# zju3dv/pats

Hardware: AMD Instinct MI355X
Metric: image-pairs/sec (coarse+fine OT) on 640x480 MegaDepth; OT iters/sec per pair (higher is better)
Workload: dtype f32 (contractions: fp32 operands split into fp16 hi + lo, three exact-product MFMA passes, fp32 accumulate)

## Files before the change

### pats_amd/csrc/gather.hip

```cpp
#include "common.hpp"

#include <cstdlib>
#include <type_traits>

namespace pats {

template <int POL, typename T>
__device__ __forceinline__ T ldm(const T* p) {
    if (POL & 1) return __builtin_nontemporal_load(p);
    return *p;
}
template <int POL, typename T>
__device__ __forceinline__ void stm(T* p, T v) {
    if (POL & 2) __builtin_nontemporal_store(v, p);
    else *p = v;
}

typedef float f2u __attribute__((ext_vector_type(2), aligned(4)));
template <int POL>
__device__ __forceinline__ f2u ldm2(const float* p) {
    const f2u* q = reinterpret_cast<const f2u*>(p);
    if (POL & 1) return __builtin_nontemporal_load(q);
    return *q;
}

template <int DT> struct map_elem { using type = uint16_t; };
template <> struct map_elem<PATS_MAP_F32> { using type = float; };
template <int DT> using map_t = typename map_elem<DT>::type;

template <int DT>
__device__ __forceinline__ float widen(uint32_t h) {
    if (DT == PATS_MAP_BF16) return __uint_as_float(h << 16);
    return (float)__builtin_bit_cast(_Float16, (uint16_t)h);
}
template <int DT>
__device__ __forceinline__ float widen_hi(uint32_t h) {
    if (DT == PATS_MAP_BF16) return __uint_as_float(h & 0xffff0000u);
    return (float)__builtin_bit_cast(_Float16, (uint16_t)(h >> 16));
}
typedef uint32_t u32u __attribute__((aligned(2)));
template <int POL>
__device__ __forceinline__ uint32_t ldh2(const uint16_t* p) {
    const u32u* q = reinterpret_cast<const u32u*>(p);
    if (POL & 1) return __builtin_nontemporal_load(q);
    return *q;
}
typedef uint32_t u4 __attribute__((ext_vector_type(4)));
typedef float f2s __attribute__((ext_vector_type(2), aligned(4)));
template <int POL>
__device__ __forceinline__ void stm2(float* p, f2s v) {
    f2s* q = reinterpret_cast<f2s*>(p);
    if (POL & 2) __builtin_nontemporal_store(v, q);
    else *q = v;
}

template <int OT> using out_t = map_t<OT>;
template <int OT>
__device__ __forceinline__ out_t<OT> narrow(float v) {
    if constexpr (OT == PATS_MAP_F32) return v;
    else if constexpr (OT == PATS_MAP_F16) return __builtin_bit_cast(uint16_t, (_Float16)v);
    else return __builtin_bit_cast(uint16_t, (__bf16)v);
}
template <int OT>
__device__ __forceinline__ uint32_t narrow2(float lo, float hi) {
    return (uint32_t)narrow<OT>(lo) | ((uint32_t)narrow<OT>(hi) << 16);
}
template <int POL>
__device__ __forceinline__ void sth2(uint16_t* p, uint32_t v) {
    u32u* q = reinterpret_cast<u32u*>(p);
    if (POL & 2) __builtin_nontemporal_store(v, q);
    else *q = v;
}
template <int OT>
__device__ __forceinline__ u4 narrow8(const float* t) {
    typedef float f4 __attribute__((ext_vector_type(4)));
    const f4 a = *reinterpret_cast<const f4*>(t), b = *reinterpret_cast<const f4*>(t + 4);
    u4 r;
    r.x = narrow2<OT>(a.x, a.y); r.y = narrow2<OT>(a.z, a.w);
    r.z = narrow2<OT>(b.x, b.y); r.w = narrow2<OT>(b.z, b.w);
    return r;
}

template <int DT, int POL>
__device__ __forceinline__ float pooled_tap(const map_t<DT>* q, int row) {
    if constexpr (DT == PATS_MAP_F32) {
        const f2u a = ldm2<POL>(q), c2 = ldm2<POL>(q + row);
        return (((a.x + a.y) + c2.x) + c2.y) / 4.0f;
    } else {
        const uint32_t a = ldh2<POL>(q), c2 = ldh2<POL>(q + row);
        return (((widen<DT>(a) + widen_hi<DT>(a)) + widen<DT>(c2)) + widen_hi<DT>(c2)) / 4.0f;
    }
}
template <int DT, int POL>
__device__ __forceinline__ float single_tap(const map_t<DT>* q) {
    if constexpr (DT == PATS_MAP_F32) return ldm<POL>(q);
    else return widen<DT>(ldm<POL>(q));
}

template <int DT, int POL, int OT>
__global__ void __launch_bounds__(256)
fine_desc_kernel(const map_t<DT>* __restrict__ f0, const map_t<DT>* __restrict__ f1,
                 const map_t<DT>* __restrict__ f2, const float* __restrict__ title,
                 const float* __restrict__ rubbish, int64_t B, out_t<OT>* __restrict__ desc,
                 const int64_t* __restrict__ B_live) {
    const int64_t n = blockIdx.x;
    const int64_t b = n % B;
    if (B_live && b >= *B_live) return;
    const int lane = threadIdx.x & 63, wave = threadIdx.x >> 6;
    out_t<OT>* o = desc + n * 264 * 145;
    int pt[3], off0[3], off1[3];
    bool live[3];
#pragma unroll
    for (int g = 0; g < 3; ++g) {
        const int p = OT == PATS_MAP_F32 ? lane + 64 * g : (g < 2 ? 2 * lane + g : 128 + lane);
        live[g] = p < 145;
        pt[g] = p < 144 ? p : 0;
        const int r = pt[g] / 12, c = pt[g] - r * 12;
        off0[g] = (4 * r + 1) * 48 + 4 * c + 1;
        off1[g] = (2 * r) * 24 + 2 * c;
    }
    const bool dust = lane == 16;
    auto put = [&](int ch, float v0, float v1, float v2) {
        out_t<OT>* row = o + ch * 145;
        if constexpr (OT == PATS_MAP_F32) {
            stm<POL>(row + lane, v0);
            stm<POL>(row + lane + 64, v1);
            if (live[2]) stm<POL>(row + lane + 128, dust ? rubbish[b * 264 + ch] : v2);
        } else {
            sth2<POL>(row + 2 * lane, narrow2<OT>(v0, v1));
            if (live[2]) stm<POL>(row + lane + 128, narrow<OT>(dust ? rubbish[b * 264 + ch] : v2));
        }
    };
    for (int ch = wave; ch < 8; ch += 4) {
        const float v = title[b * 8 + ch];
        put(ch, v, v, v);
    }
#pragma unroll 2
    for (int ch = 8 + wave; ch < 72; ch += 4) {
        const map_t<DT>* m = f0 + (n * 64 + (ch - 8)) * 48 * 48;
        float v[3];
#pragma unroll
        for (int g = 0; g < 3; ++g) v[g] = pooled_tap<DT, POL>(m + off0[g], 48);
        put(ch, v[0], v[1], v[2]);
    }
#pragma unroll 2
    for (int ch = 72 + wave; ch < 136; ch += 4) {
        const map_t<DT>* m = f1 + (n * 64 + (ch - 72)) * 24 * 24;
        float v[3];
#pragma unroll
        for (int g = 0; g < 3; ++g) v[g] = pooled_tap<DT, POL>(m + off1[g], 24);
        put(ch, v[0], v[1], v[2]);
    }
#pragma unroll 4
    for (int ch = 136 + wave; ch < 264; ch += 4) {
        const map_t<DT>* m = f2 + (n * 128 + (ch - 136)) * 144;
        put(ch, single_tap<DT, POL>(m + pt[0]), single_tap<DT, POL>(m + pt[1]), single_tap<DT, POL>(m + pt[2]));
    }
}

__device__ __forceinline__ long long round_half_even_div(float x, float d) {
    return (long long)rintf(x / d);
}

struct third_point {
    long long i00[2], bb2, i2;
};
__device__ __forceinline__ third_point third_point_at(const float* __restrict__ mk0, const float* __restrict__ mk1,
                                                      int64_t p, int64_t b, int64_t B, bool write,
                                                      int64_t* __restrict__ ps_out, int64_t* __restrict__ pt_out) {
    constexpr int W = 8, M = 52;
    const long long s0 = round_half_even_div(mk0[p * 2 + 0], 4.0f) * 4, s1 = round_half_even_div(mk0[p * 2 + 1], 4.0f) * 4;
    float t0 = mk1[p * 2 + 0], t1 = mk1[p * 2 + 1];
    t0 = t0 >= 96.f ? 96.f : t0; t1 = t1 >= 96.f ? 96.f : t1;
    t0 = t0 <= 0.f ? 0.f : t0;   t1 = t1 <= 0.f ? 0.f : t1;
    const long long q0 = round_half_even_div(t0, 4.0f) * 4, q1 = round_half_even_div(t1, 4.0f) * 4;
    if (write) {
        if (ps_out) { ps_out[p * 2] = s0; ps_out[p * 2 + 1] = s1; }
        if (pt_out) { pt_out[p * 2] = q0; pt_out[p * 2 + 1] = q1; }
    }
    auto fdiv2 = [](long long v) { return v >= 0 ? v / 2 : -((-v + 1) / 2); };
    third_point r;
    r.i00[0] = b * M * M + (fdiv2(s1) - W / 2 + 2) * M + (fdiv2(s0) - W / 2 + 2);
    r.i00[1] = b * M * M + (fdiv2(q1) - W / 2 + 2) * M + (fdiv2(q0) - W / 2 + 2);
    long long i2 = b * 144 + round_half_even_div((float)s1, 8.0f) * 12 + round_half_even_div((float)s0, 8.0f);
    i2 = i2 < 0 ? 0 : (i2 > B * 144 - 1 ? B * 144 - 1 : i2);
    r.bb2 = i2 / 144;
    r.i2 = i2 - r.bb2 * 144;
    return r;
}

template <int POL, int OT>
__global__ void __launch_bounds__(256)
third_desc_point_kernel(const float* __restrict__ ff0, const float* __restrict__ ff1,
                  const float* __restrict__ mk0, const float* __restrict__ mk1,
                  const int64_t* __restrict__ b_ids, const float* __restrict__ kenc,
                  const float* __restrict__ rubbish, int64_t P, int64_t B,
                  out_t<OT>* __restrict__ out0, out_t<OT>* __restrict__ out1, int64_t* __restrict__ ps_out,
                  int64_t* __restrict__ pt_out, const int64_t* __restrict__ P_dev) {
    constexpr int W = 8, M = 52, C = 128;
    int64_t live = P;
    if (P_dev) { const int64_t n = *P_dev; live = n < P ? n : P; }
    const int64_t per = (live + 7) >> 3, p = (int64_t)(blockIdx.x & 7) * per + (blockIdx.x >> 3);
    if ((int64_t)(blockIdx.x >> 3) >= per || p >= live) return;
    const int lane = threadIdx.x & 63, wave = threadIdx.x >> 6;
    const int64_t b = b_ids[p];
    const third_point tp = third_point_at(mk0, mk1, p, b, B, threadIdx.x == 0, ps_out, pt_out);
    const int wx = lane % W, wy = lane / W;
    long long i0 = tp.i00[0] + wy * M + wx, i1 = tp.i00[1] + wy * M + wx;
    const long long lim = B * M * M - 1;
    i0 = i0 < 0 ? 0 : (i0 > lim ? lim : i0);
    i1 = i1 < 0 ? 0 : (i1 > lim ? lim : i1);
    const long long bb0 = i0 / (M * M), r0 = i0 - bb0 * (M * M);
    const long long bb1 = i1 / (M * M), r1 = i1 - bb1 * (M * M);
    out_t<OT>* o0 = out0 + p * C * 65;
    out_t<OT>* o1 = out1 + p * C * 65;
    const float* src0 = ff0 + bb0 * C * (M * M) + r0;
    const float* src1 = ff1 + bb1 * C * (M * M) + r1;
#pragma unroll 1
    for (int c0 = 32 * wave; c0 < 32 * wave + 32; c0 += 8) {
        float a[8], c[8], ke[8];
#pragma unroll
        for (int k = 0; k < 8; ++k) {
            a[k] = ldm<POL>(src0 + (int64_t)(c0 + k) * (M * M));
            c[k] = ldm<POL>(src1 + (int64_t)(c0 + k) * (M * M));
            ke[k] = kenc[(c0 + k) * 64 + lane];
        }
#pragma unroll
        for (int k = 0; k < 8; ++k) {
            stm<POL>(o0 + (c0 + k) * 65 + lane, narrow<OT>(a[k] + ke[k]));
            stm<POL>(o1 + (c0 + k) * 65 + lane, narrow<OT>(c[k] + ke[k]));
        }
    }
    if (lane < 32) {
        const int ch = 32 * wave + lane;
        const float rb = rubbish[(tp.bb2 * C + ch) * 144 + tp.i2];
        o0[ch * 65 + 64] = narrow<OT>(rb);
        o1[ch * 65 + 64] = narrow<OT>(rb);
    }
}

constexpr int THIRD_TILE = 8;

template <int POL>
__global__ void __launch_bounds__(256)
third_desc_kernel(const float* __restrict__ ff0, const float* __restrict__ ff1,
                  const float* __restrict__ mk0, const float* __restrict__ mk1,
                  const int64_t* __restrict__ b_ids, const float* __restrict__ kenc,
                  const float* __restrict__ rubbish, int64_t P, int64_t B,
                  float* __restrict__ out0, float* __restrict__ out1, int64_t* __restrict__ ps_out,
                  int64_t* __restrict__ pt_out, const int64_t* __restrict__ P_dev) {
    constexpr int PW = THIRD_TILE / 4;
    constexpr int M = 52, C = 128, NT = 65, T = THIRD_TILE, SPAN = 8 * NT;
    typedef float f4 __attribute__((ext_vector_type(4)));
    __shared__ __attribute__((aligned(16))) float stage[4 * PW * SPAN];
    int64_t live = P;
    if (P_dev) { const int64_t n = *P_dev; live = n < P ? n : P; }
    const int64_t tiles = (live + T - 1) / T, per = (tiles + 7) >> 3, tile = (int64_t)(blockIdx.x & 7) * per + (blockIdx.x >> 3);
    if ((int64_t)(blockIdx.x >> 3) >= per || tile >= tiles) return;
    const int lane = threadIdx.x & 63, wave = __builtin_amdgcn_readfirstlane(threadIdx.x >> 6);
    const long long lim = B * M * M - 1;
    int64_t pp[PW];
    bool on[PW];
    const float* src[PW][2];
    const float* rub[PW];
#pragma unroll
    for (int j = 0; j < PW; ++j) {
        const int64_t p = tile * T + wave * PW + j;
        on[j] = p < live;
        pp[j] = on[j] ? p : live - 1;
        const int64_t b = b_ids[pp[j]];
        const third_point tp = third_point_at(mk0, mk1, pp[j], b, B, on[j] && lane == 0, ps_out, pt_out);
#pragma unroll
        for (int s = 0; s < 2; ++s) {
            long long i = tp.i00[s] + (lane >> 3) * M + (lane & 7);
            i = i < 0 ? 0 : (i > lim ? lim : i);
            const long long bb = i / (M * M);
            src[j][s] = (s ? ff1 : ff0) + bb * C * (M * M) + (i - bb * (M * M));
        }
        rub[j] = rubbish + tp.bb2 * C * 144 + tp.i2;
    }
    float* slice = stage + wave * PW * SPAN;
#pragma unroll 1
    for (int c0 = 0; c0 < C; c0 += 8) {
        float a[PW][2][8], ke[8], rb[PW];
#pragma unroll
        for (int k = 0; k < 8; ++k) {
#pragma unroll
            for (int j = 0; j < PW; ++j) {
                a[j][0][k] = ldm<POL>(src[j][0] + (int64_t)(c0 + k) * (M * M));
                a[j][1][k] = ldm<POL>(src[j][1] + (int64_t)(c0 + k) * (M * M));
            }
            ke[k] = kenc[(c0 + k) * 64 + lane];
        }
#pragma unroll
        for (int j = 0; j < PW; ++j) rb[j] = lane < 8 ? rub[j][(c0 + lane) * 144] : 0.f;
#pragma unroll
        for (int j = 0; j < PW; ++j) {
            float* sl = slice + j * SPAN;
#pragma unroll
            for (int s = 0; s < 2; ++s) {
#pragma unroll
                for (int k = 0; k < 8; ++k) sl[k * NT + lane] = a[j][s][k] + ke[k];
                if (lane < 8) sl[lane * NT + 64] = rb[j];
                wave_lds_sync();
                const f4* v = reinterpret_cast<const f4*>(sl);
                f4* o = reinterpret_cast<f4*>((s ? out1 : out0) + pp[j] * (C * NT) + c0 * NT);
                if (on[j]) {
                    stm<POL>(o + lane, v[lane]);
                    stm<POL>(o + lane + 64, v[lane + 64]);
                    if (lane < SPAN / 4 - 128) stm<POL>(o + lane + 128, v[lane + 128]);
                }
                wave_lds_sync();
            }
        }
    }
}

template <int DT, int POL, int OT>
__global__ void __launch_bounds__(256)
third_desc_half_kernel(const uint16_t* __restrict__ ff0, const uint16_t* __restrict__ ff1,
                       const float* __restrict__ mk0, const float* __restrict__ mk1,
                       const int64_t* __restrict__ b_ids, const float* __restrict__ kenc,
                       const float* __restrict__ rubbish, int64_t P, int64_t B,
                       out_t<OT>* __restrict__ out0, out_t<OT>* __restrict__ out1, int64_t* __restrict__ ps_out,
                       int64_t* __restrict__ pt_out, const int64_t* __restrict__ P_dev) {
    constexpr int M = 52, C = 128;
    int64_t live = P;
    if (P_dev) { const int64_t n = *P_dev; live = n < P ? n : P; }
    const int64_t per = (live + 7) >> 3, p = (int64_t)(blockIdx.x & 7) * per + (blockIdx.x >> 3);
    if ((int64_t)(blockIdx.x >> 3) >= per || p >= live) return;
    const int lane = threadIdx.x & 63, wave = threadIdx.x >> 6;
    const int cp = lane & 31, sub = lane >> 5;
    const int64_t b = b_ids[p];
    const third_point tp = third_point_at(mk0, mk1, p, b, B, threadIdx.x == 0, ps_out, pt_out);
    const long long lim = B * M * M - 1;
    const uint16_t* src[2];
    bool below[2], above[2];
#pragma unroll
    for (int s = 0; s < 2; ++s) {
        const long long i = tp.i00[s] + (cp >> 2) * M + 2 * (cp & 3);
        below[s] = i < 0;
        above[s] = i > lim;
        const long long j = below[s] ? 0 : (above[s] ? lim - 1 : i);
        const long long bb = j / (M * M);
        src[s] = (s ? ff1 : ff0) + bb * C * (M * M) + (j - bb * (M * M));
    }
    auto fix = [](uint32_t u, bool lo, bool hi) {
        u = lo ? (u & 0xffffu) * 0x10001u : u;
        return hi ? (u >> 16) * 0x10001u : u;
    };
    out_t<OT>* o0 = out0 + p * C * 65 + 2 * cp;
    out_t<OT>* o1 = out1 + p * C * 65 + 2 * cp;
#pragma unroll 1
    for (int c0 = 32 * wave + sub; c0 < 32 * wave + 32; c0 += 16) {
        uint32_t a[8], c[8];
        f2s ke[8];
#pragma unroll
        for (int k = 0; k < 8; ++k) {
            a[k] = ldm<POL>(reinterpret_cast<const uint32_t*>(src[0] + (int64_t)(c0 + 2 * k) * (M * M)));
            c[k] = ldm<POL>(reinterpret_cast<const uint32_t*>(src[1] + (int64_t)(c0 + 2 * k) * (M * M)));
            ke[k] = *reinterpret_cast<const f2s*>(kenc + (c0 + 2 * k) * 64 + 2 * cp);
        }
#pragma unroll
        for (int k = 0; k < 8; ++k) {
            const uint32_t u = fix(a[k], below[0], above[0]), v = fix(c[k], below[1], above[1]);
            f2s x, y;
            x.x = widen<DT>(u) + ke[k].x; x.y = widen_hi<DT>(u) + ke[k].y;
            y.x = widen<DT>(v) + ke[k].x; y.y = widen_hi<DT>(v) + ke[k].y;
            if constexpr (OT == PATS_MAP_F32) {
                stm2<POL>(o0 + (c0 + 2 * k) * 65, x);
                stm2<POL>(o1 + (c0 + 2 * k) * 65, y);
            } else {
                sth2<POL>(o0 + (c0 + 2 * k) * 65, narrow2<OT>(x.x, x.y));
                sth2<POL>(o1 + (c0 + 2 * k) * 65, narrow2<OT>(y.x, y.y));
            }
        }
    }
    if (lane < 32) {
        const int ch = 32 * wave + lane;
        const float rb = rubbish[(tp.bb2 * C + ch) * 144 + tp.i2];
        out0[p * C * 65 + ch * 65 + 64] = narrow<OT>(rb);
        out1[p * C * 65 + ch * 65 + 64] = narrow<OT>(rb);
    }
}



template <int DT, int POL, int OT>
__global__ void __launch_bounds__(256)
third_desc_nhwc_kernel(const map_t<DT>* __restrict__ ff0, const map_t<DT>* __restrict__ ff1,
                       const float* __restrict__ mk0, const float* __restrict__ mk1,
                       const int64_t* __restrict__ b_ids, const float* __restrict__ kenc,
                       const float* __restrict__ rubbish, int64_t P, int64_t B,
                       out_t<OT>* __restrict__ out0, out_t<OT>* __restrict__ out1, int64_t* __restrict__ ps_out,
                       int64_t* __restrict__ pt_out, const int64_t* __restrict__ P_dev) {
    constexpr int M = 52, C = 128, NT = 65;
    __shared__ __attribute__((aligned(16))) float tile[C * NT];
    int64_t live = P;
    if (P_dev) { const int64_t n = *P_dev; live = n < P ? n : P; }
    const unsigned k = blockIdx.x >> 3;
    const int side = k & 1;
    const int64_t per = (live + 7) >> 3, p = (int64_t)(blockIdx.x & 7) * per + (k >> 1);
    if ((int64_t)(k >> 1) >= per || p >= live) return;
    const int t = threadIdx.x, lane = t & 63, wave = __builtin_amdgcn_readfirstlane(t >> 6);
    const int64_t b = b_ids[p];
    const third_point tp = third_point_at(mk0, mk1, p, b, B, t == 0 && side == 0, ps_out, pt_out);
    const long long lim = B * M * M - 1;
    const map_t<DT>* __restrict__ ff = side ? ff1 : ff0;
    float rb = 0.f;
    if (t < C) rb = rubbish[(tp.bb2 * C + t) * 144 + tp.i2];
    const int cg = lane >> 2;
    std::conditional_t<DT == PATS_MAP_F32, float[2][16], u4[4]> v;
    if constexpr (DT == PATS_MAP_F32) {
#pragma unroll
        for (int j = 0; j < 16; ++j) {
            long long i = (side ? tp.i00[1] : tp.i00[0]) + (2 * wave + (j >> 3)) * M + (j & 7);
            i = i < 0 ? 0 : (i > lim ? lim : i);
            const float* src = ff + i * C;
            v[0][j] = ldm<POL>(src + lane);
            v[1][j] = ldm<POL>(src + lane + 64);
        }
    } else {
#pragma unroll
        for (int j = 0; j < 4; ++j) {
            const int cell = 16 * j + 4 * wave + (lane & 3);
            long long i = (side ? tp.i00[1] : tp.i00[0]) + (cell >> 3) * M + (cell & 7);
            i = i < 0 ? 0 : (i > lim ? lim : i);
            v[j] = ldm<POL>(reinterpret_cast<const u4*>(ff + i * C + 8 * cg));
        }
    }
    constexpr int KE = OT == PATS_MAP_F32 ? 33 : 40;
    float ke[KE];
    if constexpr (OT == PATS_MAP_F32) {
#pragma unroll
        for (int r = 0; r < 33; ++r) {
            const int e = t + 256 * r, c = e / NT, n = e - c * NT;
            ke[r] = kenc[(e < C * NT && n < 64) ? c * 64 + n : 0];
        }
    } else {
#pragma unroll
        for (int r = 0; r < 5; ++r) {
#pragma unroll
            for (int h = 0; h < 8; ++h) {
                const int e0 = 8 * (t + 256 * r), c0 = e0 / NT, n0 = e0 - c0 * NT + h;
                const int c = n0 < NT ? c0 : c0 + 1, n = n0 < NT ? n0 : n0 - NT;
                ke[8 * r + h] = kenc[(e0 < C * NT && n < 64) ? c * 64 + n : 0];
            }
        }
    }
    if constexpr (DT == PATS_MAP_F32) {
#pragma unroll
        for (int j = 0; j < 16; ++j) {
            tile[lane * NT + 16 * wave + j] = v[0][j];
            tile[(lane + 64) * NT + 16 * wave + j] = v[1][j];
        }
    } else {
#pragma unroll
        for (int j = 0; j < 4; ++j) {
            const int cell = 16 * j + 4 * wave + (lane & 3);
#pragma unroll
            for (int h = 0; h < 4; ++h) {
                tile[(8 * cg + 2 * h) * NT + cell] = widen<DT>(v[j][h]);
                tile[(8 * cg + 2 * h + 1) * NT + cell] = widen_hi<DT>(v[j][h]);
            }
        }
    }
    if (t < C) tile[t * NT + 64] = rb;
    wg_barrier();
    out_t<OT>* o = (side ? out1 : out0) + p * C * NT;
    if constexpr (OT == PATS_MAP_F32) {
#pragma unroll
        for (int r = 0; r < 33; ++r) {
            const int e = t + 256 * r, c = e / NT, n = e - c * NT;
            if (e < C * NT) stm<POL>(o + e, n < 64 ? tile[e] + ke[r] : tile[e]);
        }
    } else {
#pragma unroll
        for (int r = 0; r < 5; ++r) {
            const int q = t + 256 * r;
            if (q < C * NT / 8) {
                float x[8];
                const int n0 = (8 * q) % NT;
#pragma unroll
                for (int h = 0; h < 8; ++h)
                    x[h] = n0 + h != 64 ? tile[8 * q + h] + ke[8 * r + h] : tile[8 * q + h];
                u4 w;
                w.x = narrow2<OT>(x[0], x[1]); w.y = narrow2<OT>(x[2], x[3]);
                w.z = narrow2<OT>(x[4], x[5]); w.w = narrow2<OT>(x[6], x[7]);
                stm<POL>(reinterpret_cast<u4*>(o) + q, w);
            }
        }
    }
}

template <int DT, int TAPS, int POL, int OT>
__device__ __forceinline__ void fine_tile_pass(const map_t<DT>* __restrict__ img, int cpp, int ch0, int rowpix, int step,
                                               int first, float* tile, out_t<OT>* __restrict__ o,
                                               const float* __restrict__ rub, int t) {
    constexpr int NP = 145;
    typedef float f4 __attribute__((ext_vector_type(4)));
    float dust = 0.f;
    if (t < 64) dust = rub[t];
    if constexpr (DT == PATS_MAP_F32) {
        const int lane = t & 63, wave = t >> 6, cg = lane & 15, sub = lane >> 4;
        constexpr int GR = TAPS == 1 ? 9 : 3;
#pragma unroll 1
        for (int g0 = 0; g0 < 9; g0 += GR) {
            f4 q[GR][TAPS];
#pragma unroll
            for (int g = 0; g < GR; ++g) {
                const int nd = 16 * (g0 + g) + 4 * wave + sub, r = nd / 12, c = nd - 12 * r;
                const float* px = img + ((step * r + first) * rowpix + step * c + first) * cpp + ch0 + 4 * cg;
#pragma unroll
                for (int tap = 0; tap < TAPS; ++tap)
                    q[g][tap] = ldm<POL>(reinterpret_cast<const f4*>(px + ((tap >> 1) * rowpix + (tap & 1)) * cpp));
            }
#pragma unroll
            for (int g = 0; g < GR; ++g) {
                const int nd = 16 * (g0 + g) + 4 * wave + sub;
                f4 v = q[g][0];
                if (TAPS == 4) v = (((q[g][0] + q[g][1]) + q[g][2]) + q[g][3]) / 4.0f;
                tile[(4 * cg + 0) * NP + nd] = v.x;
                tile[(4 * cg + 1) * NP + nd] = v.y;
                tile[(4 * cg + 2) * NP + nd] = v.z;
                tile[(4 * cg + 3) * NP + nd] = v.w;
            }
        }
    } else {
        const int lane = t & 63, wave = t >> 6, cg = lane & 7, sub = lane >> 3;
        u4 q[5][TAPS];
#pragma unroll
        for (int g = 0; g < 5; ++g) {
            const int nd = 32 * g + 8 * wave + sub, r = nd / 12, c = nd - 12 * r;
            if (g < 4 || wave < 2) {
                const uint16_t* px = img + ((step * r + first) * rowpix + step * c + first) * cpp + ch0 + 8 * cg;
#pragma unroll
                for (int tap = 0; tap < TAPS; ++tap)
                    q[g][tap] = ldm<POL>(reinterpret_cast<const u4*>(px + ((tap >> 1) * rowpix + (tap & 1)) * cpp));
            }
        }
#pragma unroll
        for (int g = 0; g < 5; ++g) {
            const int nd = 32 * g + 8 * wave + sub;
            if (g < 4 || wave < 2) {
#pragma unroll
                for (int h = 0; h < 8; ++h) {
                    float v;
                    if (TAPS == 4) {
                        float x[4];
#pragma unroll
                        for (int tap = 0; tap < 4; ++tap)
                            x[tap] = h & 1 ? widen_hi<DT>(q[g][tap][h >> 1]) : widen<DT>(q[g][tap][h >> 1]);
                        v = (((x[0] + x[1]) + x[2]) + x[3]) / 4.0f;
                    } else {
                        v = h & 1 ? widen_hi<DT>(q[g][0][h >> 1]) : widen<DT>(q[g][0][h >> 1]);
                    }
                    tile[(8 * cg + h) * NP + nd] = v;
                }
            }
        }
    }
    if (t < 64) tile[t * NP + 144] = dust;
    wg_barrier();
    if constexpr (OT == PATS_MAP_F32) {
        const f4* src = reinterpret_cast<const f4*>(tile);
        f4* dst = reinterpret_cast<f4*>(o);
        for (int e = t; e < 64 * NP / 4; e += 256) stm<POL>(dst + e, src[e]);
    } else {
        u4* dst = reinterpret_cast<u4*>(o);
        for (int e = t; e < 64 * NP / 8; e += 256) stm<POL>(dst + e, narrow8<OT>(tile + 8 * e));
    }
    wg_barrier();
}

template <int DT, int POL, int OT>
__global__ void __launch_bounds__(256)
fine_desc_nhwc_kernel(const map_t<DT>* __restrict__ f0, const map_t<DT>* __restrict__ f1,
                      const map_t<DT>* __restrict__ f2, const float* __restrict__ title,
                      const float* __restrict__ rubbish, int64_t B, out_t<OT>* __restrict__ desc,
                      const int64_t* __restrict__ B_live) {
    constexpr int NP = 145;
    __shared__ __attribute__((aligned(16))) float tile[64 * NP];
    const int64_t n = blockIdx.x;
    const int64_t b = n % B;
    if (B_live && b >= *B_live) return;
    const int t = threadIdx.x;
    out_t<OT>* o = desc + n * 264 * NP;
    const float* rub = rubbish + b * 264;
    for (int e = t; e < 8 * NP; e += 256) {
        const int ch = e / NP, p = e - ch * NP;
        o[e] = narrow<OT>(p == 144 ? rub[ch] : title[b * 8 + ch]);
    }
    fine_tile_pass<DT, 4, POL, OT>(f0 + n * 48 * 48 * 64, 64, 0, 48, 4, 1, tile, o + 8 * NP, rub + 8, t);
    fine_tile_pass<DT, 4, POL, OT>(f1 + n * 24 * 24 * 64, 64, 0, 24, 2, 0, tile, o + 72 * NP, rub + 72, t);
    fine_tile_pass<DT, 1, POL, OT>(f2 + n * 144 * 128, 128, 0, 12, 1, 0, tile, o + 136 * NP, rub + 136, t);
    fine_tile_pass<DT, 1, POL, OT>(f2 + n * 144 * 128, 128, 64, 12, 1, 0, tile, o + 200 * NP, rub + 200, t);
}

static int gather_policy(bool channels_last) {
    static const int pol = [] { const char* e = env_switch("PATS_GATHER_NT"); return e ? (atoi(e) & 3) : -1; }();
    return pol >= 0 ? pol : (channels_last ? 3 : 0);
}

template <int V> using int_c = std::integral_constant<int, V>;
template <typename F>
static void with_gather(int dt, int ot, bool channels_last, F&& f) {
    auto pol = [&](auto d, auto o) {
        switch (gather_policy(channels_last)) {
            case 0: f(d, int_c<0>{}, o); break;
            case 1: f(d, int_c<1>{}, o); break;
            case 2: f(d, int_c<2>{}, o); break;
            default: f(d, int_c<3>{}, o); break;
        }
    };
    auto out = [&](auto d) {
        switch (ot) {
            case PATS_MAP_F16: pol(d, int_c<PATS_MAP_F16>{}); break;
            case PATS_MAP_BF16: pol(d, int_c<PATS_MAP_BF16>{}); break;
            default: pol(d, int_c<PATS_MAP_F32>{}); break;
        }
    };
    switch (dt) {
        case PATS_MAP_F16: out(int_c<PATS_MAP_F16>{}); break;
        case PATS_MAP_BF16: out(int_c<PATS_MAP_BF16>{}); break;
        default: out(int_c<PATS_MAP_F32>{}); break;
    }
}

static int launch_fine(const void* f0, const void* f1, const void* f2, int dt, bool channels_last, const float* title,
                       const float* rubbish, int64_t B, const int64_t* B_dev, void* desc, int ot, pats_stream_t stream) {
    with_gather(dt, ot, channels_last, [&](auto d, auto pol, auto o) {
        constexpr int DT = decltype(d)::value, POL = decltype(pol)::value, OT = decltype(o)::value;
        using T = map_t<DT>;
        auto go = [&](auto kernel) {
            hipLaunchKernelGGL(kernel, dim3((unsigned)(2 * B)), dim3(256), 0, as_stream(stream), (const T*)f0, (const T*)f1,
                               (const T*)f2, title, rubbish, B, (out_t<OT>*)desc, B_dev);
        };
        if (channels_last) go(fine_desc_nhwc_kernel<DT, POL, OT>);
        else go(fine_desc_kernel<DT, POL, OT>);
    });
    return check_launch(channels_last ? "fine_desc_nhwc_kernel" : "fine_desc_kernel");
}

static int g_third_gather = 0;
static int launch_third(const void* f0, const void* f1, int dt, bool channels_last, const float* mkpts0_c,
                        const float* mkpts1_c, const int64_t* b_ids, const float* kenc, const float* rubbish, int64_t P_cap,
                        const int64_t* P_dev, int64_t B, void* out0, void* out1, int ot, int64_t* p_s_out, int64_t* p_t_out,
                        pats_stream_t stream) {
    const char* name = "third_desc_nhwc_kernel";
    with_gather(dt, ot, channels_last, [&](auto d, auto pol, auto o) {
        constexpr int DT = decltype(d)::value, POL = decltype(pol)::value, OT = decltype(o)::value;
        using T = map_t<DT>;
        auto go = [&](auto kernel, const char* kname, int64_t blocks, auto* o0, auto* o1) {
            hipLaunchKernelGGL(kernel, dim3((unsigned)blocks), dim3(256), 0, as_stream(stream), (const T*)f0, (const T*)f1,
                               mkpts0_c, mkpts1_c, b_ids, kenc, rubbish, P_cap, B, o0, o1, p_s_out, p_t_out, P_dev);
            name = kname;
        };
        out_t<OT>* const o0 = (out_t<OT>*)out0;
        out_t<OT>* const o1 = (out_t<OT>*)out1;
        if (channels_last)
            go(third_desc_nhwc_kernel<DT, POL, OT>, "third_desc_nhwc_kernel", (P_cap + 7) / 8 * 16, o0, o1);
        else if constexpr (DT != PATS_MAP_F32)
            go(third_desc_half_kernel<DT, POL, OT>, "third_desc_half_kernel", (P_cap + 7) / 8 * 8, o0, o1);
        else if constexpr (OT != PATS_MAP_F32)
            go(third_desc_point_kernel<POL, OT>, "third_desc_point_kernel", (P_cap + 7) / 8 * 8, o0, o1);
        else if (g_third_gather == 1 || ((uintptr_t)out0 | (uintptr_t)out1) % 16 != 0)
            go(third_desc_point_kernel<POL, OT>, "third_desc_point_kernel", (P_cap + 7) / 8 * 8, o0, o1);
        else
            go(third_desc_kernel<POL>, "third_desc_kernel", ((P_cap + THIRD_TILE - 1) / THIRD_TILE + 7) / 8 * 8, o0, o1);
    });
    return check_launch(name);
}

}

using namespace pats;

extern "C" int pats_set_third_gather(int mode) {
    const int prev = g_third_gather;
    if (mode == 0 || mode == 1) g_third_gather = mode;
    return prev;
}

extern "C" int pats_fine_descriptors_f32(const float* feat0, const float* feat1, const float* feat2,
                                         const float* title, const float* rubbish, int64_t B,
                                         float* desc, pats_stream_t stream) {
    PATS_REQUIRE(B >= 0, "fine_descriptors: bad shape");
    if (B == 0) return PATS_OK;
    PATS_REQUIRE(feat0 && feat1 && feat2 && title && rubbish && desc, "fine_descriptors: null pointer");
    return launch_fine(feat0, feat1, feat2, PATS_MAP_F32, false, title, rubbish, B, nullptr, desc, PATS_MAP_F32, stream);
}

extern "C" int pats_fine_descriptors_counted_f32(const float* feat0, const float* feat1, const float* feat2,
                                                 const float* title, const float* rubbish, int64_t B_cap,
                                                 const int64_t* B_dev, int channels_last, float* desc, pats_stream_t stream) {
    PATS_REQUIRE(B_cap >= 0, "fine_descriptors_counted: bad shape");
    if (B_cap == 0) return PATS_OK;
    PATS_REQUIRE(B_dev && feat0 && feat1 && feat2 && title && rubbish && desc, "fine_descriptors_counted: null pointer");
    if (channels_last)
        PATS_REQUIRE(((uintptr_t)feat0 | (uintptr_t)feat1 | (uintptr_t)feat2 | (uintptr_t)desc) % 16 == 0,
                     "fine_descriptors_counted: channels-last maps and desc must be 16-byte aligned");
    return launch_fine(feat0, feat1, feat2, PATS_MAP_F32, channels_last, title, rubbish, B_cap, B_dev, desc, PATS_MAP_F32, stream);
}

extern "C" int pats_third_descriptors_f32(const float* feat_f0, const float* feat_f1,
                                          const float* mkpts0_c, const float* mkpts1_c,
                                          const int64_t* b_ids, const float* kenc, const float* rubbish,
                                          int64_t P, int64_t B, float* out0, float* out1,
                                          int64_t* p_s_out, int64_t* p_t_out, pats_stream_t stream) {
    PATS_REQUIRE(P >= 0 && B > 0, "third_descriptors: bad shape");
    if (P == 0) return PATS_OK;
    PATS_REQUIRE(feat_f0 && feat_f1 && mkpts0_c && mkpts1_c && b_ids && kenc && rubbish && out0 && out1,
                 "third_descriptors: null pointer");
    return launch_third(feat_f0, feat_f1, PATS_MAP_F32, false, mkpts0_c, mkpts1_c, b_ids, kenc, rubbish, P, nullptr, B, out0,
                        out1, PATS_MAP_F32, p_s_out, p_t_out, stream);
}

extern "C" int pats_third_descriptors_counted_f32(const float* feat_f0, const float* feat_f1,
                                                  const float* mkpts0_c, const float* mkpts1_c,
                                                  const int64_t* b_ids, const float* kenc, const float* rubbish,
                                                  int64_t P_cap, const int64_t* P_dev, int64_t B, float* out0, float* out1,
                                                  int64_t* p_s_out, int64_t* p_t_out, pats_stream_t stream) {
    PATS_REQUIRE(P_cap >= 0 && B > 0, "third_descriptors_counted: bad shape");
    if (P_cap == 0) return PATS_OK;
    PATS_REQUIRE(P_dev && feat_f0 && feat_f1 && mkpts0_c && mkpts1_c && b_ids && kenc && rubbish && out0 && out1,
                 "third_descriptors_counted: null pointer");
    return launch_third(feat_f0, feat_f1, PATS_MAP_F32, false, mkpts0_c, mkpts1_c, b_ids, kenc, rubbish, P_cap, P_dev, B, out0,
                        out1, PATS_MAP_F32, p_s_out, p_t_out, stream);
}

extern "C" int pats_fine_descriptors_nhwc_f32(const float* feat0, const float* feat1, const float* feat2,
                                              const float* title, const float* rubbish, int64_t B,
                                              float* desc, pats_stream_t stream) {
    PATS_REQUIRE(B >= 0, "fine_descriptors_nhwc: bad shape");
    if (B == 0) return PATS_OK;
    PATS_REQUIRE(feat0 && feat1 && feat2 && title && rubbish && desc, "fine_descriptors_nhwc: null pointer");
    PATS_REQUIRE(((uintptr_t)feat0 | (uintptr_t)feat1 | (uintptr_t)feat2 | (uintptr_t)desc) % 16 == 0,
                 "fine_descriptors_nhwc: maps and desc must be 16-byte aligned");
    return launch_fine(feat0, feat1, feat2, PATS_MAP_F32, true, title, rubbish, B, nullptr, desc, PATS_MAP_F32, stream);
}

extern "C" int pats_third_descriptors_nhwc_f32(const float* feat_f0, const float* feat_f1,
                                               const float* mkpts0_c, const float* mkpts1_c,
                                               const int64_t* b_ids, const float* kenc, const float* rubbish,
                                               int64_t P_cap, const int64_t* P_dev, int64_t B, float* out0, float* out1,
                                               int64_t* p_s_out, int64_t* p_t_out, pats_stream_t stream) {
    PATS_REQUIRE(P_cap >= 0 && B > 0, "third_descriptors_nhwc: bad shape");
    if (P_cap == 0) return PATS_OK;
    PATS_REQUIRE(feat_f0 && feat_f1 && mkpts0_c && mkpts1_c && b_ids && kenc && rubbish && out0 && out1,
                 "third_descriptors_nhwc: null pointer");
    return launch_third(feat_f0, feat_f1, PATS_MAP_F32, true, mkpts0_c, mkpts1_c, b_ids, kenc, rubbish, P_cap, P_dev, B, out0,
                        out1, PATS_MAP_F32, p_s_out, p_t_out, stream);
}


extern "C" int pats_fine_descriptors_typed(const void* feat0, const void* feat1, const void* feat2, pats_map_dtype_t dtype,
                                           int channels_last, const float* title, const float* rubbish, int64_t B_cap,
                                           const int64_t* B_dev, float* desc, pats_stream_t stream) {
    PATS_REQUIRE(dtype == PATS_MAP_F32 || dtype == PATS_MAP_F16 || dtype == PATS_MAP_BF16,
                 "fine_descriptors_typed: unknown map dtype %d", (int)dtype);
    PATS_REQUIRE(B_cap >= 0, "fine_descriptors_typed: bad shape");
    if (B_cap == 0) return PATS_OK;
    PATS_REQUIRE(feat0 && feat1 && feat2 && title && rubbish && desc, "fine_descriptors_typed: null pointer");
    const uintptr_t maps = (uintptr_t)feat0 | (uintptr_t)feat1 | (uintptr_t)feat2;
    if (channels_last)
        PATS_REQUIRE((maps | (uintptr_t)desc) % 16 == 0, "fine_descriptors_typed: channels-last maps and desc must be 16-byte aligned");
    else
        PATS_REQUIRE(maps % 4 == 0, "fine_descriptors_typed: NCHW maps must be 4-byte aligned");
    return launch_fine(feat0, feat1, feat2, dtype, channels_last, title, rubbish, B_cap, B_dev, desc, PATS_MAP_F32, stream);
}

extern "C" int pats_third_descriptors_typed(const void* feat_f0, const void* feat_f1, pats_map_dtype_t dtype, int channels_last,
                                            const float* mkpts0_c, const float* mkpts1_c, const int64_t* b_ids,
                                            const float* kenc, const float* rubbish, int64_t P_cap, const int64_t* P_dev,
                                            int64_t B, float* out0, float* out1, int64_t* p_s_out, int64_t* p_t_out,
                                            pats_stream_t stream) {
    PATS_REQUIRE(dtype == PATS_MAP_F32 || dtype == PATS_MAP_F16 || dtype == PATS_MAP_BF16,
                 "third_descriptors_typed: unknown map dtype %d", (int)dtype);
    PATS_REQUIRE(P_cap >= 0 && B > 0, "third_descriptors_typed: bad shape");
    if (P_cap == 0) return PATS_OK;
    PATS_REQUIRE(feat_f0 && feat_f1 && mkpts0_c && mkpts1_c && b_ids && kenc && rubbish && out0 && out1,
                 "third_descriptors_typed: null pointer");
    const uintptr_t maps = (uintptr_t)feat_f0 | (uintptr_t)feat_f1;
    if (channels_last)
        PATS_REQUIRE(maps % (dtype == PATS_MAP_F32 ? 4 : 16) == 0, "third_descriptors_typed: channels-last maps must be %d-byte aligned",
                     dtype == PATS_MAP_F32 ? 4 : 16);
    else
        PATS_REQUIRE(maps % 4 == 0, "third_descriptors_typed: NCHW maps must be 4-byte aligned");
    return launch_third(feat_f0, feat_f1, dtype, channels_last, mkpts0_c, mkpts1_c, b_ids, kenc, rubbish, P_cap, P_dev, B, out0,
                        out1, PATS_MAP_F32, p_s_out, p_t_out, stream);
}


extern "C" int pats_fine_descriptors_typed_out(const void* feat0, const void* feat1, const void* feat2, pats_map_dtype_t dtype,
                                               int channels_last, const float* title, const float* rubbish, int64_t B_cap,
                                               const int64_t* B_dev, void* desc, pats_map_dtype_t out_dtype,
                                               pats_stream_t stream) {
    PATS_REQUIRE(out_dtype == PATS_MAP_F32 || out_dtype == PATS_MAP_F16 || out_dtype == PATS_MAP_BF16,
                 "fine_descriptors_typed_out: unknown output dtype %d", (int)out_dtype);
    if (out_dtype == PATS_MAP_F32)
        return pats_fine_descriptors_typed(feat0, feat1, feat2, dtype, channels_last, title, rubbish, B_cap, B_dev, (float*)desc,
                                           stream);
    PATS_REQUIRE(dtype == PATS_MAP_F32 || dtype == PATS_MAP_F16 || dtype == PATS_MAP_BF16,
                 "fine_descriptors_typed_out: unknown map dtype %d", (int)dtype);
    PATS_REQUIRE(B_cap >= 0, "fine_descriptors_typed_out: bad shape");
    if (B_cap == 0) return PATS_OK;
    PATS_REQUIRE(feat0 && feat1 && feat2 && title && rubbish && desc, "fine_descriptors_typed_out: null pointer");
    const uintptr_t maps = (uintptr_t)feat0 | (uintptr_t)feat1 | (uintptr_t)feat2;
    if (channels_last) {
        PATS_REQUIRE((maps | (uintptr_t)desc) % 16 == 0,
                     "fine_descriptors_typed_out: channels-last maps and desc must be 16-byte aligned");
    } else {
        PATS_REQUIRE(maps % 4 == 0, "fine_descriptors_typed_out: NCHW maps must be 4-byte aligned");
        PATS_REQUIRE((uintptr_t)desc % 2 == 0, "fine_descriptors_typed_out: a half desc must be 2-byte aligned");
    }
    return launch_fine(feat0, feat1, feat2, dtype, channels_last, title, rubbish, B_cap, B_dev, desc, out_dtype, stream);
}

extern "C" int pats_third_descriptors_typed_out(const void* feat_f0, const void* feat_f1, pats_map_dtype_t dtype,
                                                int channels_last, const float* mkpts0_c, const float* mkpts1_c,
                                                const int64_t* b_ids, const float* kenc, const float* rubbish, int64_t P_cap,
                                                const int64_t* P_dev, int64_t B, void* out0, void* out1,
                                                pats_map_dtype_t out_dtype, int64_t* p_s_out, int64_t* p_t_out,
                                                pats_stream_t stream) {
    PATS_REQUIRE(out_dtype == PATS_MAP_F32 || out_dtype == PATS_MAP_F16 || out_dtype == PATS_MAP_BF16,
                 "third_descriptors_typed_out: unknown output dtype %d", (int)out_dtype);
    if (out_dtype == PATS_MAP_F32)
        return pats_third_descriptors_typed(feat_f0, feat_f1, dtype, channels_last, mkpts0_c, mkpts1_c, b_ids, kenc, rubbish, P_cap,
                                            P_dev, B, (float*)out0, (float*)out1, p_s_out, p_t_out, stream);
    PATS_REQUIRE(dtype == PATS_MAP_F32 || dtype == PATS_MAP_F16 || dtype == PATS_MAP_BF16,
                 "third_descriptors_typed_out: unknown map dtype %d", (int)dtype);
    PATS_REQUIRE(P_cap >= 0 && B > 0, "third_descriptors_typed_out: bad shape");
    if (P_cap == 0) return PATS_OK;
    PATS_REQUIRE(feat_f0 && feat_f1 && mkpts0_c && mkpts1_c && b_ids && kenc && rubbish && out0 && out1,
                 "third_descriptors_typed_out: null pointer");
    const uintptr_t maps = (uintptr_t)feat_f0 | (uintptr_t)feat_f1, outs = (uintptr_t)out0 | (uintptr_t)out1;
    if (channels_last) {
        PATS_REQUIRE(maps % (dtype == PATS_MAP_F32 ? 4 : 16) == 0,
                     "third_descriptors_typed_out: channels-last maps must be %d-byte aligned", dtype == PATS_MAP_F32 ? 4 : 16);
        PATS_REQUIRE(outs % 16 == 0, "third_descriptors_typed_out: half outputs of channels-last maps must be 16-byte aligned");
    } else {
        PATS_REQUIRE(maps % 4 == 0, "third_descriptors_typed_out: NCHW maps must be 4-byte aligned");
        PATS_REQUIRE(outs % 2 == 0, "third_descriptors_typed_out: half outputs must be 2-byte aligned");
    }
    return launch_third(feat_f0, feat_f1, dtype, channels_last, mkpts0_c, mkpts1_c, b_ids, kenc, rubbish, P_cap, P_dev, B, out0,
                        out1, out_dtype, p_s_out, p_t_out, stream);
}
```

Before: 1953.

## Batch fine-descriptor gather loads ahead of stores to raise memory-level parallelism

The NCHW fine descriptor kernel now gives each wave a contiguous block of channels and processes them in batches. All loads for a batch (pooled or single taps plus the rubbish value) are issued first, then converted and stored, with empty asm barriers keeping the loads in flight. The goal is to hide global-load latency in a gather kernel that is latency-bound, at the cost of more registers per thread. The wave index is made scalar and the old strided kernel is kept behind a diagnostic flag.

```diff
diff --git a/pats_amd/csrc/gather.hip b/pats_amd/csrc/gather.hip
--- a/pats_amd/csrc/gather.hip
+++ b/pats_amd/csrc/gather.hip
@@ -81,20 +81,47 @@
     return r;
 }
 
+template <int DT> struct pooled_raw {
+    std::conditional_t<DT == PATS_MAP_F32, f2u, uint32_t> a, c2;
+};
 template <int DT, int POL>
-__device__ __forceinline__ float pooled_tap(const map_t<DT>* q, int row) {
-    if constexpr (DT == PATS_MAP_F32) {
-        const f2u a = ldm2<POL>(q), c2 = ldm2<POL>(q + row);
-        return (((a.x + a.y) + c2.x) + c2.y) / 4.0f;
-    } else {
-        const uint32_t a = ldh2<POL>(q), c2 = ldh2<POL>(q + row);
-        return (((widen<DT>(a) + widen_hi<DT>(a)) + widen<DT>(c2)) + widen_hi<DT>(c2)) / 4.0f;
-    }
-}
-template <int DT, int POL>
-__device__ __forceinline__ float single_tap(const map_t<DT>* q) {
-    if constexpr (DT == PATS_MAP_F32) return ldm<POL>(q);
-    else return widen<DT>(ldm<POL>(q));
+__device__ __forceinline__ pooled_raw<DT> pooled_load(const map_t<DT>* q, int row) {
+    if constexpr (DT == PATS_MAP_F32) return {ldm2<POL>(q), ldm2<POL>(q + row)};
+    else return {ldh2<POL>(q), ldh2<POL>(q + row)};
+}
+template <int DT>
+__device__ __forceinline__ float pooled_value(const pooled_raw<DT>& t) {
+    if constexpr (DT == PATS_MAP_F32) return (((t.a.x + t.a.y) + t.c2.x) + t.c2.y) / 4.0f;
+    else return (((widen<DT>(t.a) + widen_hi<DT>(t.a)) + widen<DT>(t.c2)) + widen_hi<DT>(t.c2)) / 4.0f;
+}
+template <int DT>
+__device__ __forceinline__ float single_value(map_t<DT> t) {
+    if constexpr (DT == PATS_MAP_F32) return t;
+    else return widen<DT>(t);
+}
+
+template <int DT> __device__ __forceinline__ void keep_loaded(const pooled_raw<DT>& t) { asm volatile("" ::"v"(t.a), "v"(t.c2)); }
+__device__ __forceinline__ void keep_loaded(float t) { asm volatile("" ::"v"(t)); }
+__device__ __forceinline__ void keep_loaded(uint16_t t) { asm volatile("" ::"v"((uint32_t)t)); }
+
+#ifndef PATS_FINE_NB_POOLED
+#define PATS_FINE_NB_POOLED 8
+#endif
+#ifndef PATS_FINE_NB_SINGLE
+#define PATS_FINE_NB_SINGLE 16
+#endif
+
+template <int NCH, int NB, class T, class Load, class Emit>
+__device__ __forceinline__ void fine_batches(Load&& load, Emit&& emit) {
+    static_assert(NCH % NB == 0, "the batch size divides a wave's channels of the map");
+#pragma unroll 1
+    for (int k = 0; k < NCH / NB; ++k) {
+        T t[NB];
+#pragma unroll
+        for (int i = 0; i < NB; ++i) t[i] = load(k * NB + i);
+#pragma unroll
+        for (int i = 0; i < NB; ++i) emit(k * NB + i, t[i]);
+    }
 }
 
 template <int DT, int POL, int OT>
@@ -103,6 +130,81 @@
                  const map_t<DT>* __restrict__ f2, const float* __restrict__ title,
                  const float* __restrict__ rubbish, int64_t B, out_t<OT>* __restrict__ desc,
                  const int64_t* __restrict__ B_live) {
+    const int64_t n = blockIdx.x;
+    const int64_t b = n % B;
+    if (B_live && b >= *B_live) return;
+    const int lane = threadIdx.x & 63, wave = __builtin_amdgcn_readfirstlane(threadIdx.x >> 6);
+    out_t<OT>* o = desc + n * 264 * 145;
+    const float* rub = rubbish + b * 264;
+    uint32_t pt[3], off0[3], off1[3];
+    bool live[3];
+#pragma unroll
+    for (int g = 0; g < 3; ++g) {
+        const int p = OT == PATS_MAP_F32 ? lane + 64 * g : (g < 2 ? 2 * lane + g : 128 + lane);
+        live[g] = p < 145;
+        pt[g] = p < 144 ? p : 0;
+        const uint32_t r = pt[g] / 12, c = pt[g] - r * 12;
+        off0[g] = (4 * r + 1) * 48 + 4 * c + 1;
+        off1[g] = (2 * r) * 24 + 2 * c;
+    }
+    const bool dust = lane == 16;
+    auto put = [&](int ch, float v0, float v1, float v2, float rb) {
+        out_t<OT>* row = o + ch * 145;
+        if constexpr (OT == PATS_MAP_F32) {
+            stm<POL>(row + lane, v0);
+            stm<POL>(row + lane + 64, v1);
+            if (live[2]) stm<POL>(row + lane + 128, dust ? rb : v2);
+        } else {
+            sth2<POL>(row + 2 * lane, narrow2<OT>(v0, v1));
+            if (live[2]) stm<POL>(row + lane + 128, narrow<OT>(dust ? rb : v2));
+        }
+    };
+    auto chan = [&](int j, int nch) { return wave * nch + j; };
+    for (int j = 0; j < 2; ++j) {
+        const int ch = chan(j, 2);
+        const float v = title[b * 8 + ch];
+        put(ch, v, v, v, rub[ch]);
+    }
+    struct pooled_ch { pooled_raw<DT> g[3]; float rb; };
+    struct single_ch { map_t<DT> g[3]; float rb; };
+    auto pooled_map = [&](const map_t<DT>* m, uint32_t plane, int row, const uint32_t (&off)[3], int ch0) {
+        fine_batches<16, PATS_FINE_NB_POOLED, pooled_ch>(
+            [&](int j) {
+                pooled_ch t;
+#pragma unroll
+                for (int g = 0; g < 3; ++g) t.g[g] = pooled_load<DT, POL>(m + chan(j, 16) * plane + off[g], row);
+                t.rb = rub[ch0 + chan(j, 16)];
+                return t;
+            },
+            [&](int j, const pooled_ch& t) {
+                put(ch0 + chan(j, 16), pooled_value<DT>(t.g[0]), pooled_value<DT>(t.g[1]), pooled_value<DT>(t.g[2]), t.rb);
+                keep_loaded(t.g[2]);
+            });
+    };
+    pooled_map(f0 + n * 64 * 48 * 48, 48 * 48, 48, off0, 8);
+    pooled_map(f1 + n * 64 * 24 * 24, 24 * 24, 24, off1, 72);
+    const map_t<DT>* m2 = f2 + n * 128 * 144;
+    fine_batches<32, PATS_FINE_NB_SINGLE, single_ch>(
+        [&](int j) {
+            single_ch t;
+#pragma unroll
+            for (int g = 0; g < 3; ++g) t.g[g] = ldm<POL>(m2 + chan(j, 32) * 144 + pt[g]);
+            t.rb = rub[136 + chan(j, 32)];
+            return t;
+        },
+        [&](int j, const single_ch& t) {
+            put(136 + chan(j, 32), single_value<DT>(t.g[0]), single_value<DT>(t.g[1]), single_value<DT>(t.g[2]), t.rb);
+            keep_loaded(t.g[2]);
+        });
+}
+
+#ifdef PATS_DIAG
+template <int DT, int POL, int OT>
+__global__ void __launch_bounds__(256)
+fine_desc_serial_kernel(const map_t<DT>* __restrict__ f0, const map_t<DT>* __restrict__ f1,
+                        const map_t<DT>* __restrict__ f2, const float* __restrict__ title,
+                        const float* __restrict__ rubbish, int64_t B, out_t<OT>* __restrict__ desc,
+                        const int64_t* __restrict__ B_live) {
     const int64_t n = blockIdx.x;
     const int64_t b = n % B;
     if (B_live && b >= *B_live) return;
@@ -131,6 +233,7 @@
             if (live[2]) stm<POL>(row + lane + 128, narrow<OT>(dust ? rubbish[b * 264 + ch] : v2));
         }
     };
+    auto pooled_tap = [](const map_t<DT>* q, int row) { return pooled_value<DT>(pooled_load<DT, POL>(q, row)); };
     for (int ch = wave; ch < 8; ch += 4) {
         const float v = title[b * 8 + ch];
         put(ch, v, v, v);
@@ -140,7 +243,7 @@
         const map_t<DT>* m = f0 + (n * 64 + (ch - 8)) * 48 * 48;
         float v[3];
 #pragma unroll
-        for (int g = 0; g < 3; ++g) v[g] = pooled_tap<DT, POL>(m + off0[g], 48);
+        for (int g = 0; g < 3; ++g) v[g] = pooled_tap(m + off0[g], 48);
         put(ch, v[0], v[1], v[2]);
     }
 #pragma unroll 2
@@ -148,15 +251,16 @@
         const map_t<DT>* m = f1 + (n * 64 + (ch - 72)) * 24 * 24;
         float v[3];
 #pragma unroll
-        for (int g = 0; g < 3; ++g) v[g] = pooled_tap<DT, POL>(m + off1[g], 24);
+        for (int g = 0; g < 3; ++g) v[g] = pooled_tap(m + off1[g], 24);
         put(ch, v[0], v[1], v[2]);
     }
 #pragma unroll 4
     for (int ch = 136 + wave; ch < 264; ch += 4) {
         const map_t<DT>* m = f2 + (n * 128 + (ch - 136)) * 144;
-        put(ch, single_tap<DT, POL>(m + pt[0]), single_tap<DT, POL>(m + pt[1]), single_tap<DT, POL>(m + pt[2]));
-    }
-}
+        put(ch, single_value<DT>(ldm<POL>(m + pt[0])), single_value<DT>(ldm<POL>(m + pt[1])), single_value<DT>(ldm<POL>(m + pt[2])));
+    }
+}
+#endif
 
 __device__ __forceinline__ long long round_half_even_div(float x, float d) {
     return (long long)rintf(x / d);
@@ -637,6 +741,9 @@
                                (const T*)f2, title, rubbish, B, (out_t<OT>*)desc, B_dev);
         };
         if (channels_last) go(fine_desc_nhwc_kernel<DT, POL, OT>);
+#ifdef PATS_DIAG
+        else if (diag_env("PATS_FINE_SERIAL")) go(fine_desc_serial_kernel<DT, POL, OT>);
+#endif
         else go(fine_desc_kernel<DT, POL, OT>);
     });
     return check_launch(channels_last ? "fine_desc_nhwc_kernel" : "fine_desc_kernel");
```

Measured after the change: 1950. No clear change (-0.1%).
